# hmchuong/MaGGIe

Measured on AMD Instinct MI355X. Metric: instance-frames/sec (fwd+bwd+optimizer step, 512x512, bf16), higher is better.
Workload: dtype bf16

## Files before the change

### include/maggie_hip.h

```cpp
#ifndef MAGGIE_HIP_H
#define MAGGIE_HIP_H
#include <stdint.h>
#ifdef __cplusplus
extern "C" {
#endif

#define MG_F32 0
#define MG_BF16 1
#define MG_F16 3

#define MG_ACT_NONE 0
#define MG_ACT_RELU 1
#define MG_ACT_LRELU 2

#define MG_STAT_REPLICAS 32

#define MG_MODE_CONV 0
#define MG_MODE_TCONV 1
#define MG_MODE_GATHER 2

int mg_abi_version(void);
int mg_set_zeroed_range(void* base, long bytes);
int mg_zero_claim(void* p, long bytes);
int mg_zeroed_range_conflicts(void);
// ... 160 lines not shown
int mg_attn_tok_bwd(const float* p, const float* feat, const float* qk, const int32_t* ids, const float* dctx, const float* dp, int B, int T,
                    int L, int D, int NID, float scale, float* gbuf, float* rowdot, float* dqk, float* dbtab, float* dfeat, void* stream);
int mg_attn_feat_fwd(const float* feat, const float* kq, const float* b2, const float* vp, const float* obias, const uint8_t* pad_mask,
                     const int32_t* ids, int B, int T, int L, int D, int NID, float scale, float* out, float* p, void* stream);
int mg_attn_feat_bwd(const float* dout, const float* p, const float* feat, const float* kq, const float* vp, const int32_t* ids, int B, int T,
                     int L, int D, int NID, float scale, float* dfeat, float* dkq, float* dvp, float* db2, float* dobias, void* stream);
int mg_attn_feat_fwd_ex(const float* feat, const float* kq, const float* b2, const float* vp, const float* obias, const uint8_t* pad_mask,
                        const int32_t* ids, int B, int T, int L, int Dm, int NID, float scale, float* out, float* p, int b2_tn, void* stream);
int mg_attn_feat_bwd_ex(const float* dout, const float* p, const float* feat, const float* kq, const float* vp, const int32_t* ids, int B, int T,
                        int L, int Dm, int NID, float scale, float* dfeat, float* dkq, float* dvp, float* db2, float* dobias, int b2_tn, void* stream);

int mg_plane_flags(const float* w, int P, int HW, int32_t* flags, void* stream);
int mg_plane_flags_ex(const float* w, int P, int HW, void* flags, int as_float, void* stream);
int mg_os8_weight(const float* gt, const float* a8, int P, long HW, int reweight, int32_t* flags_scratch, float* out, void* stream);
int mg_os8_weight_ex(const float* gt, const float* a8, int P, long HW, int reweight, int32_t* flags_scratch, float* out, const int32_t* pvalid,
                     void* stream);
int mg_loss_finish(const float* sums, float* out3, void* stream);
int mg_loss_coef(const float* g3, const float* sums, float* coef5, void* stream);
int mg_loss_point_fwd(const float* p, const float* t, const float* w, const int32_t* flags, int P, int H, int W, float* d,
                      float* sums, const int32_t* pvalid, void* stream);
int mg_pyr_down(const float* x, const int32_t* flags, int P, int h, int w, float* out, void* stream);
int mg_pyr_lap_fwd(const float* x, const float* down, const float* w0, int lvl, int H0, int W0, const int32_t* flags, int P, int h,
                   int w, float* G, float* sums, void* stream);
int mg_pyr_upT(const float* q, const float* coef, const float* add, const int32_t* flags, int P, int h, int w, float* r, void* stream);
int mg_pyr_downT(const float* r, const float* q, const float* coef, const int32_t* flags, int P, int h, int w, float* dd, void* stream);
int mg_loss_point_bwd(const float* p, const float* t, const float* w, const int32_t* flags, int P, int H, int W, const float* coef_rec,
                      const float* coef_grad, const float* dd, float* A, float* B, float* dp, const int32_t* pvalid, void* stream);

int mg_matting_losses_fwd(const float* const* p, const float* t, const float* const* w, const int32_t* pvalid, int S, int P, int H, int W, int32_t* flags,
                          float* d, float* down0, float* down1, float* down2, float* G0, float* G1, float* G2, float* sums, float* out, void* stream);
int mg_matting_losses_bwd(const float* g, const float* sums, const float* const* p, const float* t, const float* const* w, const int32_t* pvalid,
                          const int32_t* flags, int S, int P, int H, int W, const float* G0, const float* G1, const float* G2, float* coef, float* r2,
                          float* dd2, float* r1, float* dd1, float* r0, float* dd0, float* A, float* B, float* dp, void* stream);

typedef struct mg_sn_desc {
    const float* W;
    float* u;
    float* v;
    int64_t out_off;
    int64_t work_off;
    int64_t dw_off;
    int32_t A, B, taps, transposed, pad_in;
    int32_t plain;
    int32_t k3_first, k3_count;
} mg_sn_desc;
int mg_spectral_norm_batched(const mg_sn_desc* descs, int n_conv, const int32_t* items_k1, int n1, const int32_t* items_k2, int n2,
                             const int32_t* items_k3, int n3, float* work_base, long work_floats, void* out_base, void* out_t_base,
                             int out_dtype, void* stream);
int mg_spectral_norm_batched_bwd(const mg_sn_desc* descs, int n_conv, const int32_t* items_k3, int n3, const void* const* Gptrs,
                                 int g_dtype, float* work_base, float* dW_base, float* dot_part, void* stream);
int mg_spectral_norm_batched_bwd_to(const mg_sn_desc* descs, int n_conv, const int32_t* items_k3, int n3, const void* const* Gptrs,
                                    int g_dtype, float* work_base, float* dW_base, float* const* dWptrs, float* dot_part, void* stream);

int mg_gru_gate_fwd(const void* rz, const void* x, const void* h, int dtype, int M, int C, void* xrh, void* stream);
int mg_gru_gate_bwd(const void* dxrh, const void* rz, const void* h, int dtype, int M, int C, void* dx, void* drz, void* dh_part, void* stream);
int mg_gru_out_fwd(const void* rz, const void* cpre, const void* h, int dtype, int M, int C, void* hn, void* stream);
int mg_gru_out_bwd(const void* dhn, const void* rz, const void* cpre, const void* h, int dtype, int M, int C, void* drz, void* dc_pre,
                   void* dh_part, void* stream);
int mg_temporal_fuse(float* alphas, const float* prev, const float* df, const float* db, long plane_elems, int n_frames, void* stream);

#define MG_WB_MAX_ENTRIES 64
typedef struct mg_wb_entry {
    const void* src;
    void* dst;
    void* dst_t;
    int32_t cout, taps, cin, cout_pad, cin_pad, flip_t, dtype, reserved;
// ... 399 lines not shown
```

### maggie_amd/csrc/loss_stencils.h

```cpp
#pragma once

MG_STENCIL_FN int st_refl(int k, int n) { return k < 0 ? -k : (k >= n ? 2 * (n - 1) - k : k); }
MG_STENCIL_FN int st_clampi(int k, int n) { return k < 0 ? 0 : (k >= n ? n - 1 : k); }

#define MG_G1 {1.f / 16.f, 4.f / 16.f, 6.f / 16.f, 4.f / 16.f, 1.f / 16.f}

MG_STENCIL_FN bool ring_map(int t, int nh, int nw, int T, int Bt, int Lw, int Rw, int& a, int& b) {
    const int hi = nh - T - Bt, wi = nw - Lw - Rw;
    if (hi <= 0 || wi <= 0) { a = t / nw; b = t - a * nw; return false; }
    const int n_int = hi * wi;
    if (t < n_int) { const int r = t / wi; a = T + r; b = Lw + (t - r * wi); return true; }
    int u = t - n_int;
    const int n_tb = (T + Bt) * nw;
    if (u < n_tb) { const int r = u / nw; a = r < T ? r : nh - Bt + (r - T); b = u - r * nw; return false; }
    u -= n_tb;
    const int side = Lw + Rw;
    const int r = u / side, k = u - r * side;
    a = T + r; b = k < Lw ? k : nw - Rw + (k - Lw);
    return false;
}

MG_STENCIL_FN float lap_up_general(const float* __restrict__ dp, int y, int xx, int h, int w, int wd) {
    const float g[5] = MG_G1;
    int yy[5], xs[5];
// ... 15 lines not shown
        }
        up += g[i] * r;
    }
    return up;
}
MG_STENCIL_FN void lap_up_inner(const float* __restrict__ dp, int a, int b, int wd, float* up) {
    const float* __restrict__ r0 = dp + (a - 1) * wd + (b - 1);
    float d[3][3];
#pragma unroll
    for (int r = 0; r < 3; ++r)
#pragma unroll
        for (int c = 0; c < 3; ++c) d[r][c] = r0[r * wd + c];
    const float g0 = 1.f / 16.f, g1 = 4.f / 16.f, g2 = 6.f / 16.f, g3 = 4.f / 16.f, g4 = 1.f / 16.f;
    float u = 0.f;
    u += g0 * (g0 * d[0][0] + g2 * d[0][1] + g4 * d[0][2]);
    u += g2 * (g0 * d[1][0] + g2 * d[1][1] + g4 * d[1][2]);
    u += g4 * (g0 * d[2][0] + g2 * d[2][1] + g4 * d[2][2]);
    up[0] = u;
    u = 0.f;
    u += g0 * (g1 * d[0][1] + g3 * d[0][2]);
    u += g2 * (g1 * d[1][1] + g3 * d[1][2]);
    u += g4 * (g1 * d[2][1] + g3 * d[2][2]);
    up[1] = u;
    u = 0.f;
    u += g1 * (g0 * d[1][0] + g2 * d[1][1] + g4 * d[1][2]);
    u += g3 * (g0 * d[2][0] + g2 * d[2][1] + g4 * d[2][2]);
    up[2] = u;
    u = 0.f;
    u += g1 * (g1 * d[1][1] + g3 * d[1][2]);
    u += g3 * (g1 * d[2][1] + g3 * d[2][2]);
    up[3] = u;
}

MG_STENCIL_FN float upT_general(const float* __restrict__ qp, int a, int b, int h, int w) {
    const float g[5] = MG_G1;
    float acc = 0.f;
#pragma unroll
    for (int sa = 0; sa < 3; ++sa) {
        int ma = sa == 0 ? 2 * a : (sa == 1 ? -2 * a : 2 * (h - 1) - 2 * a);
        if (sa == 1 && a != 1) continue;
        if (sa == 2 && ma != h) continue;
#pragma unroll
        for (int i = 0; i < 5; ++i) {
            int y = ma - i + 2;
            if (y < 0 || y >= h) continue;
            float v[3][5];
            bool ok[3][5];
#pragma unroll
            for (int sb = 0; sb < 3; ++sb) {
                const int mb = sb == 0 ? 2 * b : (sb == 1 ? -2 * b : 2 * (w - 1) - 2 * b);
                const bool on = !(sb == 1 && b != 1) && !(sb == 2 && mb != w);
#pragma unroll
                for (int j = 0; j < 5; ++j) {
                    const int xq = mb - j + 2;
                    ok[sb][j] = on && xq >= 0 && xq < w;
                    v[sb][j] = qp[y * w + (xq < 0 ? 0 : (xq >= w ? w - 1 : xq))];
                }
            }
            float rowacc = 0.f;
#pragma unroll
            for (int sb = 0; sb < 3; ++sb)
#pragma unroll
                for (int j = 0; j < 5; ++j) {
                    if (ok[sb][j]) rowacc += g[j] * v[sb][j];
                }
            acc += g[i] * rowacc;
// ... 94 lines not shown
            int x = X + dx;
            if (x < 0 || x >= W) continue;
            float av = Ap[y * W + x], bv = Bp[y * W + x];
#pragma unroll
            for (int i = 0; i < 3; ++i) {
                if (st_clampi(y + i - 1, H) != Y) continue;
#pragma unroll
                for (int j = 0; j < 3; ++j) {
                    if (st_clampi(x + j - 1, W) != X) continue;
                    acc += kx[i][j] * av + kx[j][i] * bv;
                }
            }
        }
    }
    return acc;
}
MG_STENCIL_FN float sobel_adj_inner(const float* __restrict__ Ap, const float* __restrict__ Bp, int Y, int X, int W) {
    const float kx[3][3] = {{-1.f, 0.f, 1.f}, {-2.f, 0.f, 2.f}, {-1.f, 0.f, 1.f}};
    float a[3][3], b[3][3];
#pragma unroll
    for (int dy = 0; dy < 3; ++dy)
#pragma unroll
        for (int dx = 0; dx < 3; ++dx) {
            a[dy][dx] = Ap[(Y + dy - 1) * W + (X + dx - 1)];
            b[dy][dx] = Bp[(Y + dy - 1) * W + (X + dx - 1)];
        }
    float acc = 0.f;
#pragma unroll
    for (int dy = 0; dy < 3; ++dy)
#pragma unroll
        for (int dx = 0; dx < 3; ++dx) acc += kx[2 - dy][2 - dx] * a[dy][dx] + kx[2 - dx][2 - dy] * b[dy][dx];
    return acc;
}
```

### maggie_amd/csrc/losses.hip

```cpp
#include "common.h"
#include "launch.h"
#include "../../include/maggie_hip.h"

namespace {

#define MG_STENCIL_FN __device__ __forceinline__
#include "loss_stencils.h"

constexpr int NT = 256;
__device__ __constant__ float c_g1[5] = {1.f / 16.f, 4.f / 16.f, 6.f / 16.f, 4.f / 16.f, 1.f / 16.f};

__device__ __forceinline__ int refl(int k, int n) { return k < 0 ? -k : (k >= n ? 2 * (n - 1) - k : k); }
__device__ __forceinline__ int clampi(int k, int n) { return k < 0 ? 0 : (k >= n ? n - 1 : k); }

constexpr int LOSS_REPLICAS = 32, LOSS_STRIDE = 16;
struct P3 { const float* a[3]; };
constexpr int LOSS_SUMS = LOSS_REPLICAS * LOSS_STRIDE;

__device__ __forceinline__ void block_add(float v, float* dst, float* sh, float* slot = nullptr) {
    v = wave_sum(v);
    const int lane = threadIdx.x & 63, wave = threadIdx.x >> 6;
    if (lane == 0) sh[wave] = v;
    __syncthreads();
    if (threadIdx.x == 0) {
// ... 34 lines not shown
    if (__syncthreads_or(any) && threadIdx.x == 0) flags[p] = 1;
}

__global__ __launch_bounds__(NT) void os8_weight_kernel(const float* __restrict__ gt, const float* __restrict__ a8, const int* __restrict__ flags,
                                                        long HW, int reweight, float* __restrict__ out, const int* __restrict__ pvalid) {
    const int p = blockIdx.y;
    const float valid = flags[p] ? 1.f : 0.f;
    const float pv = (pvalid && !pvalid[p]) ? 0.f : 1.f;
    const long base = (long)p * HW;
    const float lo = 1.0f / 255.0f, hi = 254.0f / 255.0f;
    for (long i = (long)blockIdx.x * NT + threadIdx.x; i < HW; i += (long)gridDim.x * NT) {
        float w = valid;
        if (reweight) {
            const float g = gt[base + i], a = a8[base + i] * pv;
            if ((g <= hi && g >= lo) || (a <= hi && a >= lo)) w += 1.f;
        }
        out[base + i] = w;
    }
}

__device__ __forceinline__ float sobel_mag(const float* __restrict__ a, const float* __restrict__ w, int y, int x, int H, int W, float& gx,
                                           float& gy, float as = 1.f) {
    float v[3][3];
#pragma unroll
    for (int i = 0; i < 3; ++i)
#pragma unroll
        for (int j = 0; j < 3; ++j) {
            int yy = clampi(y + i - 1, H), xx = clampi(x + j - 1, W);
            v[i][j] = a[yy * W + xx] * as * w[yy * W + xx];
        }
    gx = ((v[0][2] - v[0][0]) + 2.f * (v[1][2] - v[1][0]) + (v[2][2] - v[2][0])) * 0.125f;
    gy = ((v[2][0] - v[0][0]) + 2.f * (v[2][1] - v[0][1]) + (v[2][2] - v[0][2])) * 0.125f;
    return sqrtf(gx * gx + gy * gy + 1e-6f);
}

__global__ __launch_bounds__(NT) void point_fwd_kernel(const P3 p, const float* __restrict__ t, const P3 w,
                                                       const int* __restrict__ flags, int H, int W, float* __restrict__ d,
                                                       float* __restrict__ sums, const int* __restrict__ pvalid, int Pper, float* __restrict__ slots) {
    __shared__ float sh[NT / 64];
    const int pl = blockIdx.y;
    float* slot = slots ? slots + ((size_t)blockIdx.y * gridDim.x + blockIdx.x) * 3 : nullptr;
    if (!flags[pl]) { if (slot && threadIdx.x < 3) slot[threadIdx.x] = 0.f; return; }
    const int sc = pl / Pper, pq = pl - sc * Pper;
    const float pv = (pvalid && !pvalid[pq]) ? 0.f : 1.f;
    const long off = (long)pl * H * W, offq = (long)pq * H * W;
    const float *pp = p.a[sc] + offq, *tp = t + offq, *wp = w.a[sc] + offq;
    float s0 = 0.f, s1 = 0.f, s2 = 0.f;
    for (int i = blockIdx.x * NT + threadIdx.x; i < H * W; i += gridDim.x * NT) {
        int y = i / W, x = i - y * W;
        float dv = pp[i] * pv - tp[i], wv = wp[i];
        d[off + i] = dv;
        s0 += wv * fabsf(dv);
        s2 += wv;
        float gx, gy;
        float mp = sobel_mag(pp, wp, y, x, H, W, gx, gy, pv);
        float mt = sobel_mag(tp, wp, y, x, H, W, gx, gy);
        s1 += fabsf(mp - mt);
    }
    float* srep = sums + sc * LOSS_SUMS + ((blockIdx.y * gridDim.x + blockIdx.x) & (LOSS_REPLICAS - 1)) * LOSS_STRIDE;
    block_add(s0, &srep[0], sh, slot);
    block_add(s1, &srep[1], sh, slot ? slot + 1 : nullptr);
    block_add(s2, &srep[2], sh, slot ? slot + 2 : nullptr);
}

__global__ __launch_bounds__(NT) void pyr_down_kernel(const float* __restrict__ x, const int* __restrict__ flags, int h, int w,
                                                      float* __restrict__ out) {
// ... 41 lines not shown
            const float g1[5] = {1.f / 16.f, 4.f / 16.f, 6.f / 16.f, 4.f / 16.f, 1.f / 16.f};
            const int i0 = y & 1, j0 = xx & 1;
            const float* row = dp + ((y + i0 - 2) >> 1) * wd + ((xx + j0 - 2) >> 1);
            if (j0 == 0) {
                for (int i = i0; i < 5; i += 2, row += wd) up += g1[i] * (g1[0] * row[0] + g1[2] * row[1] + g1[4] * row[2]);
            } else {
                for (int i = i0; i < 5; i += 2, row += wd) up += g1[i] * (g1[1] * row[0] + g1[3] * row[1]);
            }
        } else {
#pragma unroll
            for (int i = 0; i < 5; ++i) {
                int yy = refl(y + i - 2, h);
                if (yy & 1) continue;
                float r = 0.f;
#pragma unroll
                for (int j = 0; j < 5; ++j) {
                    int xs = refl(xx + j - 2, w);
                    if (!(xs & 1)) r += c_g1[j] * dp[(yy >> 1) * wd + (xs >> 1)];
                }
                up += c_g1[i] * r;
            }
        }
        float L = xp[o] - 4.f * up;
        float wl = wp[(long)(y << lvl) * W0 + (xx << lvl)];
        s0 += fabsf(L) * wl;
        s1 += wl;
        G[(long)pl * h * w + o] = L > 0.f ? wl : (L < 0.f ? -wl : 0.f);
    }
    float* srep = sums + sc * LOSS_SUMS + ((blockIdx.y * gridDim.x + blockIdx.x) & (LOSS_REPLICAS - 1)) * LOSS_STRIDE;
    block_add(s0, &srep[0], sh, slot);
    block_add(s1, &srep[1], sh, slot ? slot + 1 : nullptr);
}

__global__ __launch_bounds__(NT) void pyr_upT_kernel(const float* __restrict__ q, const float* __restrict__ coef, const float* __restrict__ add,
                                                     const int* __restrict__ flags, int h, int w, float* __restrict__ r, int Pper) {
    const int pl = blockIdx.y;
    if (!flags[pl]) return;
    const int hd = h >> 1, wd = w >> 1;
    const float* qp = q + (long)pl * h * w;
    const float c = coef[(pl / Pper) * 5];
    for (int o = blockIdx.x * NT + threadIdx.x; o < hd * wd; o += gridDim.x * NT) {
        int a = o / wd, b = o - a * wd;
        float acc = 0.f;
#pragma unroll
        for (int sa = 0; sa < 3; ++sa) {
            int ma = sa == 0 ? 2 * a : (sa == 1 ? -2 * a : 2 * (h - 1) - 2 * a);
            if (sa == 1 && a != 1) continue;
            if (sa == 2 && ma != h) continue;
#pragma unroll
            for (int i = 0; i < 5; ++i) {
                int y = ma - i + 2;
                if (y < 0 || y >= h) continue;
                float rowacc = 0.f;
#pragma unroll
                for (int sb = 0; sb < 3; ++sb) {
                    int mb = sb == 0 ? 2 * b : (sb == 1 ? -2 * b : 2 * (w - 1) - 2 * b);
                    if (sb == 1 && b != 1) continue;
                    if (sb == 2 && mb != w) continue;
#pragma unroll
                    for (int j = 0; j < 5; ++j) {
                        int x = mb - j + 2;
                        if (x < 0 || x >= w) continue;
                        rowacc += c_g1[j] * qp[y * w + x];
                    }
                }
                acc += c_g1[i] * rowacc;
// ... 17 lines not shown
#pragma unroll
        for (int sa = 0; sa < 3; ++sa) {
            int my = sa == 0 ? Y : (sa == 1 ? -Y : 2 * (h - 1) - Y);
            if (sa == 1 && !(Y == 1 || Y == 2)) continue;
            if (sa == 2 && !(Y == h - 2 || Y == h - 3)) continue;
#pragma unroll
            for (int i = 0; i < 5; ++i) {
                int ty = my - i + 2;
                if (ty < 0 || (ty & 1)) continue;
                int y = ty >> 1;
                if (y >= hd) continue;
                float rowacc = 0.f;
#pragma unroll
                for (int sb = 0; sb < 3; ++sb) {
                    int mx = sb == 0 ? X : (sb == 1 ? -X : 2 * (w - 1) - X);
                    if (sb == 1 && !(X == 1 || X == 2)) continue;
                    if (sb == 2 && !(X == w - 2 || X == w - 3)) continue;
#pragma unroll
                    for (int j = 0; j < 5; ++j) {
                        int tx = mx - j + 2;
                        if (tx < 0 || (tx & 1)) continue;
                        int x = tx >> 1;
                        if (x >= wd) continue;
                        rowacc += c_g1[j] * rp[y * wd + x];
                    }
                }
                acc += c_g1[i] * rowacc;
            }
        }
        dd[(long)pl * h * w + o] = c * q[(long)pl * h * w + o] + acc;
    }
}

__global__ __launch_bounds__(NT) void pyr_lap_fwd_quad_kernel(const float* __restrict__ x, const float* __restrict__ down, const P3 w0,
                                                              int lvl, int H0, int W0, const int* __restrict__ flags, int h, int w,
                                                              float* __restrict__ G, float* __restrict__ sums, int Pper, float* __restrict__ slots) {
    __shared__ float sh[NT / 64];
    const int pl = blockIdx.y;
    float* slot = slots ? slots + ((size_t)blockIdx.y * gridDim.x + blockIdx.x) * 2 : nullptr;
    if (!flags[pl]) { if (slot && threadIdx.x < 2) slot[threadIdx.x] = 0.f; return; }
    const int sc = pl / Pper;
    const int hd = h >> 1, wd = w >> 1;
    const float* __restrict__ xp = x + (long)pl * h * w;
    const float* __restrict__ dp = down + (long)pl * hd * wd;
    const float* __restrict__ wp = w0.a[sc] + (long)(pl - sc * Pper) * H0 * W0;
    float* __restrict__ Gp = G + (long)pl * h * w;
    float s0 = 0.f, s1 = 0.f;
    const int hi = hd - 2, wi = wd - 2;
    const int n_int = (hi > 0 && wi > 0) ? hi * wi : 0;
    const int total = n_int + 4 * (hd * wd - n_int);
    for (int q = blockIdx.x * NT + threadIdx.x; q < total; q += gridDim.x * NT) {
        if (q >= n_int) {
            const int bt = q - n_int;
            int a, b;
            ring_map(n_int + (bt >> 2), hd, wd, 1, 1, 1, 1, a, b);
            const int y = 2 * a + ((bt >> 1) & 1), xx = 2 * b + (bt & 1);
            const float xv1 = xp[(long)y * w + xx];
            const float wl1 = wp[(long)(y << lvl) * W0 + (xx << lvl)];
            const float L = xv1 - 4.f * lap_up_general(dp, y, xx, h, w, wd);
            s0 += fabsf(L) * wl1;
            s1 += wl1;
            Gp[(long)y * w + xx] = L > 0.f ? wl1 : (L < 0.f ? -wl1 : 0.f);
            continue;
        }
        int a, b;
        ring_map(q, hd, wd, 1, 1, 1, 1, a, b);
        const int y0 = 2 * a, x0 = 2 * b;
        const float* __restrict__ xr0 = xp + (long)y0 * w + x0;
        const float xv[4] = {xr0[0], xr0[1], xr0[w], xr0[w + 1]};
        const long wr0 = (long)(y0 << lvl) * W0, wr1 = (long)((y0 + 1) << lvl) * W0;
        const int wc0 = x0 << lvl, wc1 = (x0 + 1) << lvl;
        const float wl[4] = {wp[wr0 + wc0], wp[wr0 + wc1], wp[wr1 + wc0], wp[wr1 + wc1]};
        float up[4];
        lap_up_inner(dp, a, b, wd, up);
        float gq[4];
#pragma unroll
        for (int u = 0; u < 4; ++u) {
            const float L = xv[u] - 4.f * up[u];
            s0 += fabsf(L) * wl[u];
            s1 += wl[u];
            gq[u] = L > 0.f ? wl[u] : (L < 0.f ? -wl[u] : 0.f);
        }
        float* __restrict__ gr0 = Gp + (long)y0 * w + x0;
        gr0[0] = gq[0]; gr0[1] = gq[1]; gr0[w] = gq[2]; gr0[w + 1] = gq[3];
    }
    float* srep = sums + sc * LOSS_SUMS + ((blockIdx.y * gridDim.x + blockIdx.x) & (LOSS_REPLICAS - 1)) * LOSS_STRIDE;
    block_add(s0, &srep[0], sh, slot);
    block_add(s1, &srep[1], sh, slot ? slot + 1 : nullptr);
}

__global__ __launch_bounds__(NT) void pyr_upT_batched_kernel(const float* __restrict__ q, const float* __restrict__ coef, const float* __restrict__ add,
                                                             const int* __restrict__ flags, int h, int w, float* __restrict__ r, int Pper) {
    const int pl = blockIdx.y;
    if (!flags[pl]) return;
    const int hd = h >> 1, wd = w >> 1;
    const float* __restrict__ qp = q + (long)pl * h * w;
    const float c = coef[(pl / Pper) * 5];
    for (int o = blockIdx.x * NT + threadIdx.x; o < hd * wd; o += gridDim.x * NT) {
        int a, b;
        const bool inner = ring_map(o, hd, wd, 2, 1, 2, 1, a, b);
        const long oo = (long)pl * hd * wd + a * wd + b;
        const float base = add ? add[oo] : 0.f;
        const float acc = inner ? upT_inner(qp, a, b, w) : upT_general(qp, a, b, h, w);
        r[oo] = base - 4.f * c * acc;
    }
}

__global__ __launch_bounds__(NT) void pyr_downT_quad_kernel(const float* __restrict__ r, const float* __restrict__ q, const float* __restrict__ coef,
                                                            const int* __restrict__ flags, int h, int w, float* __restrict__ dd, int Pper) {
    const int pl = blockIdx.y;
    if (!flags[pl]) return;
    const int hd = h >> 1, wd = w >> 1;
    const float* __restrict__ rp = r + (long)pl * hd * wd;
    const float* __restrict__ qp = q + (long)pl * h * w;
    float* __restrict__ op = dd + (long)pl * h * w;
    const float c = coef[(pl / Pper) * 5];
    const int hi = hd - 4, wi = wd - 4;
    const int n_int = (hi > 0 && wi > 0) ? hi * wi : 0;
    const int total = n_int + 4 * (hd * wd - n_int);
    for (int t = blockIdx.x * NT + threadIdx.x; t < total; t += gridDim.x * NT) {
        if (t >= n_int) {
            const int bt = t - n_int;
            int a, b;
            ring_map(n_int + (bt >> 2), hd, wd, 2, 2, 2, 2, a, b);
            const int Y = 2 * a + ((bt >> 1) & 1), X = 2 * b + (bt & 1);
            const float qv1 = qp[(long)Y * w + X];
            op[(long)Y * w + X] = c * qv1 + downT_general(rp, Y, X, h, w, hd, wd);
            continue;
        }
        int a, b;
        ring_map(t, hd, wd, 2, 2, 2, 2, a, b);
        const int y0 = 2 * a, x0 = 2 * b;
        const float* __restrict__ qr0 = qp + (long)y0 * w + x0;
        const float qv[4] = {qr0[0], qr0[1], qr0[w], qr0[w + 1]};
        float acc[4];
        downT_inner(rp, a, b, wd, acc);
        float* __restrict__ o0 = op + (long)y0 * w + x0;
        o0[0] = c * qv[0] + acc[0]; o0[1] = c * qv[1] + acc[1]; o0[w] = c * qv[2] + acc[2]; o0[w + 1] = c * qv[3] + acc[3];
    }
}

__global__ __launch_bounds__(NT) void sobel_bwd1_kernel(const P3 p, const float* __restrict__ t, const P3 w,
                                                        const int* __restrict__ flags, int H, int W, float* __restrict__ A, float* __restrict__ B,
                                                        const int* __restrict__ pvalid, int Pper) {
    const int pl = blockIdx.y;
    if (!flags[pl]) return;
    const int sc = pl / Pper, pq = pl - sc * Pper;
    if (pvalid && !pvalid[pq]) return;
    const long off = (long)pl * H * W, offq = (long)pq * H * W;
    const float *pp = p.a[sc] + offq, *tp = t + offq, *wp = w.a[sc] + offq;
    for (int i = blockIdx.x * NT + threadIdx.x; i < H * W; i += gridDim.x * NT) {
        int y = i / W, x = i - y * W;
        float gx, gy, tx, ty;
        float mp = sobel_mag(pp, wp, y, x, H, W, gx, gy);
        float mt = sobel_mag(tp, wp, y, x, H, W, tx, ty);
        float s = mp > mt ? 1.f : (mp < mt ? -1.f : 0.f);
        A[off + i] = s * gx / mp;
        B[off + i] = s * gy / mp;
    }
}

__global__ __launch_bounds__(NT) void point_bwd_kernel(const P3 p, const float* __restrict__ t, const P3 w,
                                                       const int* __restrict__ flags, int H, int W, const float* __restrict__ coef_rec,
                                                       const float* __restrict__ coef_grad, const float* __restrict__ dd,
                                                       const float* __restrict__ A, const float* __restrict__ B, float* __restrict__ dp,
                                                       const int* __restrict__ pvalid, int Pper) {
    const int pl = blockIdx.y;
    const int sc = pl / Pper, pq = pl - sc * Pper;
    const long off = (long)pl * H * W, offq = (long)pq * H * W;
    if (!flags[pl] || (pvalid && !pvalid[pq])) {
        for (int idx = blockIdx.x * NT + threadIdx.x; idx < H * W; idx += gridDim.x * NT) dp[off + idx] = 0.f;
        return;
    }
    const float cr = coef_rec[sc * 5], cg = coef_grad[sc * 5];
    const float* __restrict__ pp = p.a[sc] + offq;
    const float* __restrict__ tp = t + offq;
    const float* __restrict__ wp = w.a[sc] + offq;
    const float kx[3][3] = {{-1.f, 0.f, 1.f}, {-2.f, 0.f, 2.f}, {-1.f, 0.f, 1.f}};
    for (int idx = blockIdx.x * NT + threadIdx.x; idx < H * W; idx += gridDim.x * NT) {
        int Y = idx / W, X = idx - Y * W;
        float dv = pp[idx] - tp[idx];
        float wv = wp[idx];
        float g = cr * wv * (dv > 0.f ? 1.f : (dv < 0.f ? -1.f : 0.f));
        if (dd) g += dd[off + idx];
        float acc = 0.f;
#pragma unroll
        for (int dy = -1; dy <= 1; ++dy) {
            int y = Y + dy;
// ... 20 lines not shown

__global__ __launch_bounds__(NT) void point_bwd_batched_kernel(const P3 p, const float* __restrict__ t, const P3 w,
                                                               const int* __restrict__ flags, int H, int W, const float* __restrict__ coef_rec,
                                                               const float* __restrict__ coef_grad, const float* __restrict__ dd,
                                                               const float* __restrict__ A, const float* __restrict__ B, float* __restrict__ dp,
                                                               const int* __restrict__ pvalid, int Pper) {
    const int pl = blockIdx.y;
    const int sc = pl / Pper, pq = pl - sc * Pper;
    const long off = (long)pl * H * W, offq = (long)pq * H * W;
    if (!flags[pl] || (pvalid && !pvalid[pq])) {
        for (int idx = blockIdx.x * NT + threadIdx.x; idx < H * W; idx += gridDim.x * NT) dp[off + idx] = 0.f;
        return;
    }
    const float cr = coef_rec[sc * 5], cg = coef_grad[sc * 5];
    const float* __restrict__ pp = p.a[sc] + offq;
    const float* __restrict__ tp = t + offq;
    const float* __restrict__ wp = w.a[sc] + offq;
    const float* __restrict__ Ap = A + off;
    const float* __restrict__ Bp = B + off;
    for (int idx = blockIdx.x * NT + threadIdx.x; idx < H * W; idx += gridDim.x * NT) {
        int Y, X;
        const bool inner = ring_map(idx, H, W, 1, 1, 1, 1, Y, X);
        const int px = Y * W + X;
        const float dv = pp[px] - tp[px];
        const float wv = wp[px];
        const float ddv = dd ? dd[off + px] : 0.f;
        const float acc = inner ? sobel_adj_inner(Ap, Bp, Y, X, W) : sobel_adj_general(Ap, Bp, Y, X, H, W);
        float g = cr * wv * (dv > 0.f ? 1.f : (dv < 0.f ? -1.f : 0.f));
        if (dd) g += ddv;
        dp[off + px] = g + cg * wv * acc * 0.125f;
    }
}

inline dim3 grid2(long per_plane, int P, long max_blocks = 1024) {
    long b = (per_plane + NT - 1) / NT;
    if (b > max_blocks) b = max_blocks;
    if (b < 1) b = 1;
    return dim3((unsigned)b, (unsigned)P);
}
static const long REDUCING_BLOCKS_PER_PLANE = mg_env_long("MG_LOSS_BLOCKS", 256l);

static const int LOSS_BATCHED = (int)mg_env_long("MG_LOSS_BATCHED", 1);

static void launch_pyr_lap_fwd(dim3 g, hipStream_t st, const float* x, const float* down, P3 ww, int lvl, int H0, int W0, const int* flags, int h, int w,
                               float* G, float* sums, int Pper, float* slots) {
    if (LOSS_BATCHED && !(h & 1) && !(w & 1))
        hipLaunchKernelGGL(pyr_lap_fwd_quad_kernel, g, dim3(NT), 0, st, x, down, ww, lvl, H0, W0, flags, h, w, G, sums, Pper, slots);
    else
        hipLaunchKernelGGL(pyr_lap_fwd_kernel, g, dim3(NT), 0, st, x, down, ww, lvl, H0, W0, flags, h, w, G, sums, Pper, slots);
}
static void launch_pyr_upT(int SP, hipStream_t st, const float* q, const float* coef, const float* add, const int* flags, int h, int w, float* r, int Pper) {
    const dim3 g = grid2((long)(h / 2) * (w / 2), SP);
    if (LOSS_BATCHED && !(h & 1) && !(w & 1))
        hipLaunchKernelGGL(pyr_upT_batched_kernel, g, dim3(NT), 0, st, q, coef, add, flags, h, w, r, Pper);
    else
        hipLaunchKernelGGL(pyr_upT_kernel, g, dim3(NT), 0, st, q, coef, add, flags, h, w, r, Pper);
}
static void launch_pyr_downT(int SP, hipStream_t st, const float* r, const float* q, const float* coef, const int* flags, int h, int w, float* dd, int Pper) {
    if (LOSS_BATCHED && !(h & 1) && !(w & 1))
        hipLaunchKernelGGL(pyr_downT_quad_kernel, grid2((long)(h / 2) * (w / 2), SP), dim3(NT), 0, st, r, q, coef, flags, h, w, dd, Pper);
    else
        hipLaunchKernelGGL(pyr_downT_kernel, grid2((long)h * w, SP), dim3(NT), 0, st, r, q, coef, flags, h, w, dd, Pper);
}
static void launch_point_bwd(int SP, hipStream_t st, P3 pp, const float* t, P3 ww, const int* flags, int H, int W, const float* coef_rec,
                             const float* coef_grad, const float* dd, const float* A, const float* B, float* dp, const int* pvalid, int Pper) {
    if (LOSS_BATCHED)
        hipLaunchKernelGGL(point_bwd_batched_kernel, grid2((long)H * W, SP), dim3(NT), 0, st, pp, t, ww, flags, H, W, coef_rec, coef_grad, dd, A, B, dp, pvalid, Pper);
    else
        hipLaunchKernelGGL(point_bwd_kernel, grid2((long)H * W, SP), dim3(NT), 0, st, pp, t, ww, flags, H, W, coef_rec, coef_grad, dd, A, B, dp, pvalid, Pper);
}

__device__ __forceinline__ void loss_sum_replicas(const float* __restrict__ rep, float* s) {
    if (threadIdx.x < LOSS_STRIDE) {
        float a = 0.f;
        for (int r = 0; r < LOSS_REPLICAS; ++r) a += rep[r * LOSS_STRIDE + threadIdx.x];
// ... 135 lines not shown
extern "C" int mg_matting_losses_fwd(const float* const* p, const float* t, const float* const* w, const int32_t* pvalid, int S, int P, int H, int W,
                                     int32_t* flags, float* d, float* down0, float* down1, float* down2, float* G0, float* G1, float* G2, float* sums,
                                     float* out, void* stream) {
    if (S < 1 || S > 3 || P <= 0) return -2;
    if ((H & 7) || (W & 7) || H < 16 || W < 16) return -2;
    hipStream_t st = (hipStream_t)stream;
    P3 pp{{nullptr, nullptr, nullptr}}, ww{{nullptr, nullptr, nullptr}};
    for (int i = 0; i < S; ++i) { pp.a[i] = p[i]; ww.a[i] = w[i]; }
    const int SP = S * P;
    hipError_t e = mg_zero_words(flags, (long)SP, st); if (e != hipSuccess) return (int)e;
    e = mg_zero_words(sums, (long)S * LOSS_SUMS, st); if (e != hipSuccess) return (int)e;
    { dim3 g = grid2((long)H * W, SP); if (g.x > 64) g.x = 64; hipLaunchKernelGGL(plane_flags3_kernel, g, dim3(NT), 0, st, ww, P, H * W, flags); }
    {
        const dim3 g = grid2((long)H * W, SP, REDUCING_BLOCKS_PER_PLANE);
        float* slots; int rc = loss_slots(g, 3, &slots); if (rc) return rc;
        hipLaunchKernelGGL(point_fwd_kernel, g, dim3(NT), 0, st, pp, t, ww, flags, H, W, d, sums, pvalid, P, slots);
        rc = loss_slot_reduce(slots, g, S, 3, sums, 0, st); if (rc) return rc;
    }
    const float* x = d; float* downs[3] = {down0, down1, down2}; float* Gs[3] = {G0, G1, G2};
    int h = H, wd = W;
    for (int lvl = 0; lvl < 3; ++lvl) {
        hipLaunchKernelGGL(pyr_down_kernel, grid2((long)(h / 2) * (wd / 2), SP), dim3(NT), 0, st, x, flags, h, wd, downs[lvl]);
        const dim3 g = grid2((long)h * wd, SP, REDUCING_BLOCKS_PER_PLANE);
        float* slots; int rc = loss_slots(g, 2, &slots); if (rc) return rc;
        launch_pyr_lap_fwd(g, st, x, (const float*)downs[lvl], ww, lvl, H, W, flags, h, wd, Gs[lvl], sums + 3 + 2 * lvl, P, slots);
        rc = loss_slot_reduce(slots, g, S, 2, sums, 3 + 2 * lvl, st); if (rc) return rc;
        x = downs[lvl]; h >>= 1; wd >>= 1;
    }
    hipLaunchKernelGGL(loss_finish_kernel, dim3(S), dim3(64), 0, st, (const float*)sums, out);
    MG_CHECK_LAUNCH();
    return 0;
}

extern "C" int mg_matting_losses_bwd(const float* g, const float* sums, const float* const* p, const float* t, const float* const* w,
                                     const int32_t* pvalid, const int32_t* flags, int S, int P, int H, int W, const float* G0, const float* G1,
                                     const float* G2, float* coef, float* r2, float* dd2, float* r1, float* dd1, float* r0, float* dd0, float* A, float* B,
                                     float* dp, void* stream) {
    if (S < 1 || S > 3 || P <= 0) return -2;
    hipStream_t st = (hipStream_t)stream;
    P3 pp{{nullptr, nullptr, nullptr}}, ww{{nullptr, nullptr, nullptr}};
    for (int i = 0; i < S; ++i) { pp.a[i] = p[i]; ww.a[i] = w[i]; }
    const int SP = S * P;
    hipLaunchKernelGGL(loss_coef_kernel, dim3(S), dim3(64), 0, st, g, sums, coef);
    launch_pyr_upT(SP, st, G2, (const float*)(coef + 4), (const float*)nullptr, flags, H / 4, W / 4, r2, P);
    launch_pyr_downT(SP, st, (const float*)r2, G2, (const float*)(coef + 4), flags, H / 4, W / 4, dd2, P);
    launch_pyr_upT(SP, st, G1, (const float*)(coef + 3), (const float*)dd2, flags, H / 2, W / 2, r1, P);
    launch_pyr_downT(SP, st, (const float*)r1, G1, (const float*)(coef + 3), flags, H / 2, W / 2, dd1, P);
    launch_pyr_upT(SP, st, G0, (const float*)(coef + 2), (const float*)dd1, flags, H, W, r0, P);
    launch_pyr_downT(SP, st, (const float*)r0, G0, (const float*)(coef + 2), flags, H, W, dd0, P);
    hipLaunchKernelGGL(sobel_bwd1_kernel, grid2((long)H * W, SP), dim3(NT), 0, st, pp, t, ww, flags, H, W, A, B, pvalid, P);
    launch_point_bwd(SP, st, pp, t, ww, flags, H, W, (const float*)coef, (const float*)(coef + 1), (const float*)dd0, (const float*)A, (const float*)B, dp, pvalid, P);
    MG_CHECK_LAUNCH();
    return 0;
}

__global__ __launch_bounds__(NT) void atten_loss_rows_kernel(const float* __restrict__ gm, const float* __restrict__ att, long L, float* __restrict__ terms) {
    __shared__ float sh[2 * (NT / 64)];
    const long base = (long)blockIdx.x * L;
    float sv = 0.f, sg = 0.f;
    for (long i = threadIdx.x; i < L; i += NT) { const float g = gm[base + i]; sv += g * att[base + i]; sg += g; }
    sv = wave_sum(sv); sg = wave_sum(sg);
    const int lane = threadIdx.x & 63, wave = threadIdx.x >> 6;
    if (lane == 0) { sh[wave] = sv; sh[NT / 64 + wave] = sg; }
    __syncthreads();
    if (threadIdx.x == 0) {
        float a = 0.f, b = 0.f;
        for (int w = 0; w < NT / 64; ++w) { a += sh[w]; b += sh[NT / 64 + w]; }
        terms[blockIdx.x] = (b != 0.f ? 1.f : 0.f) - a;
    }
}
__global__ void atten_loss_sum_kernel(const float* __restrict__ terms, int rows, float scale, float* __restrict__ out) {
    float s = 0.f;
    for (int i = threadIdx.x; i < rows; i += 64) s += terms[i];
    s = wave_sum(s);
    if (threadIdx.x == 0) out[0] = s * scale;
}
// ... 45 lines not shown
```

### maggie_amd/functional.py

```python
import os

import torch
import torch.distributed as dist

from . import kernels as K
from .kernels import MODE_CONV, MODE_TCONV, MODE_GATHER, ACT_NONE, ACT_RELU, ACT_LRELU

LRELU_SLOPE = 0.2
import os as _os
UNFUSED_STATS_ROWS = int(_os.environ.get('MAGGIE_UNFUSED_STATS_ROWS', str(1 << 19)))
EXACT_STATS_ROWS = int(_os.environ.get('MAGGIE_EXACT_STATS_ROWS', '32768'))


class ZeroArena:

    def __init__(self):
        self.buf = None
        self.off = 0
        self.used = 0
        self.need = 1 << 20
        self.cap_buf = None
        self.cap_off = 0
        self.spills = 0
        self.tally = 0
# ... 1391 lines not shown
        t = target.detach().float().contiguous()
        P = ps[0].numel() // (H * W_)
        dev = t.device
        K.hip.need_cuda(t, *ps, *ws)
        if pvalid is not None:
            assert pvalid.dtype == torch.int32 and pvalid.numel() == P and pvalid.is_contiguous()
        SP = S * P
        new = lambda hh, ww: torch.empty((SP, hh, ww), dtype=torch.float32, device=dev)
        flags = ARENA.acc(SP, dev, torch.int32)
        sums = ARENA.acc(S * 512, dev)
        d, downs = new(H, W_), [new(H >> 1, W_ >> 1), new(H >> 2, W_ >> 2), new(H >> 3, W_ >> 3)]
        Gs = [new(H, W_), new(H >> 1, W_ >> 1), new(H >> 2, W_ >> 2)]
        out = torch.empty((S, 3), dtype=torch.float32, device=dev)
        parr = (K.ctypes.c_void_p * S)(*[x.data_ptr() for x in ps])
        warr = (K.ctypes.c_void_p * S)(*[x.data_ptr() for x in ws])
        ptr = K.hip.ptr
        K.hip.call('mg_matting_losses_fwd', parr, ptr(t), warr, ptr(pvalid), K.c_int(S), K.c_int(P), K.c_int(H), K.c_int(W_), ptr(flags), ptr(d),
                   ptr(downs[0]), ptr(downs[1]), ptr(downs[2]), ptr(Gs[0]), ptr(Gs[1]), ptr(Gs[2]), ptr(sums), ptr(out), K.hip.stream())
        ctx.save_for_backward(t, flags, sums, *Gs, *ps, *ws)
        ctx.pvalid, ctx.S, ctx.shape = pvalid, S, preds[0].shape
        return out

    @staticmethod
    def backward(ctx, g):
        S = ctx.S
        saved = ctx.saved_tensors
        t, flags, sums, G0, G1, G2 = saved[:6]
        ps, ws = saved[6:6 + S], saved[6 + S:6 + 2 * S]
        SP, H, W_ = G0.shape
        P = SP // S
        dev = t.device
        new = lambda hh, ww: torch.empty((SP, hh, ww), dtype=torch.float32, device=dev)
        coef = torch.empty((S, 5), dtype=torch.float32, device=dev)
        r2, dd2, r1, dd1 = new(H >> 3, W_ >> 3), new(H >> 2, W_ >> 2), new(H >> 2, W_ >> 2), new(H >> 1, W_ >> 1)
        r0, dd0, A, B, dp = new(H >> 1, W_ >> 1), new(H, W_), new(H, W_), new(H, W_), new(H, W_)
        parr = (K.ctypes.c_void_p * S)(*[x.data_ptr() for x in ps])
        warr = (K.ctypes.c_void_p * S)(*[x.data_ptr() for x in ws])
        ptr = K.hip.ptr
        K.hip.call('mg_matting_losses_bwd', ptr(g.float().contiguous()), ptr(sums), parr, ptr(t), warr, ptr(ctx.pvalid), ptr(flags), K.c_int(S), K.c_int(P),
                   K.c_int(H), K.c_int(W_), ptr(G0), ptr(G1), ptr(G2), ptr(coef), ptr(r2), ptr(dd2), ptr(r1), ptr(dd1), ptr(r0), ptr(dd0), ptr(A), ptr(B),
                   ptr(dp), K.hip.stream())
        dps = tuple(dp[i * P:(i + 1) * P].view(ctx.shape) for i in range(S))
        return (None, None) + dps + (None,) * S


def matting_losses_multi(preds, target, weights, pvalid=None):
    if not LOSS_MULTI or len(preds) == 1 or len(preds) > 3:
        return [matting_losses(p_, target, w_, pvalid) for p_, w_ in zip(preds, weights)]
    out = MattingLossesMulti.apply(target, pvalid, *preds, *weights)
    cells = SplitGrid.apply(out)
    n = out.shape[1]
    return [cells[i * n:(i + 1) * n] for i in range(out.shape[0])]


class SplitGrid(torch.autograd.Function):

    @staticmethod
    def forward(ctx, t):
        ctx.set_materialize_grads(False)
        ctx.shape = t.shape
        return tuple(t[i, j] for i in range(t.shape[0]) for j in range(t.shape[1]))

    @staticmethod
    def backward(ctx, *gs):
        R, C = ctx.shape
        g0 = gs[0]
        if g0 is not None and all(g is not None and g.dtype == torch.float32 and g.numel() == 1 and g.is_cuda and
                                  g.untyped_storage().data_ptr() == g0.untyped_storage().data_ptr() and g.data_ptr() == g0.data_ptr() + 4 * i
# ... 698 lines not shown
```

Measured before the change: 773.6.

## Fuse matting-loss backward pyramid transposes and Sobel/point gradient into tiled kernels

Replaces the separate upT/downT launches of the Laplacian-pyramid backward with a combined updownT kernel per level. It also fuses the Sobel adjoint (A/B maps) and point-loss backward into one shared-memory tiled kernel that stages pred, target and weight tiles with halos. This removes intermediate dd and A/B buffers along with several kernel launches and full-resolution memory round trips. The cost is more complex tiled code with halo recomputation, plus FP-contraction pragmas intended to keep rounding consistent with the unfused path.

Result: no change. 767.2 (-0.8%).

```diff
diff --git a/include/maggie_hip.h b/include/maggie_hip.h
--- a/include/maggie_hip.h
+++ b/include/maggie_hip.h
@@ -216,6 +216,8 @@
 int mg_matting_losses_bwd(const float* g, const float* sums, const float* const* p, const float* t, const float* const* w, const int32_t* pvalid,
                           const int32_t* flags, int S, int P, int H, int W, const float* G0, const float* G1, const float* G2, float* coef, float* r2,
                           float* dd2, float* r1, float* dd1, float* r0, float* dd0, float* A, float* B, float* dp, void* stream);
+int mg_set_loss_fused(int on);
+int mg_matting_losses_bwd_fused(int H, int W);
 
 typedef struct mg_sn_desc {
     const float* W;
diff --git a/maggie_amd/csrc/loss_stencils.h b/maggie_amd/csrc/loss_stencils.h
--- a/maggie_amd/csrc/loss_stencils.h
+++ b/maggie_amd/csrc/loss_stencils.h
@@ -71,6 +71,10 @@
     up[3] = u;
 }
 
+#if defined(__clang__)
+#pragma clang fp contract(on)
+#endif
+
 MG_STENCIL_FN float upT_general(const float* __restrict__ qp, int a, int b, int h, int w) {
     const float g[5] = MG_G1;
     float acc = 0.f;
@@ -231,3 +235,148 @@
         for (int dx = 0; dx < 3; ++dx) acc += kx[2 - dy][2 - dx] * a[dy][dx] + kx[2 - dx][2 - dy] * b[dy][dx];
     return acc;
 }
+MG_STENCIL_FN float sobel_adj_general_at(const float* __restrict__ Ap, const float* __restrict__ Bp, int Y, int X, int H, int W, int oy, int ox,
+                                         int stride) {
+    const float kx[3][3] = {{-1.f, 0.f, 1.f}, {-2.f, 0.f, 2.f}, {-1.f, 0.f, 1.f}};
+    float acc = 0.f;
+#pragma unroll
+    for (int dy = -1; dy <= 1; ++dy) {
+        int y = Y + dy;
+        if (y < 0 || y >= H) continue;
+#pragma unroll
+        for (int dx = -1; dx <= 1; ++dx) {
+            int x = X + dx;
+            if (x < 0 || x >= W) continue;
+            float av = Ap[(y - oy) * stride + (x - ox)], bv = Bp[(y - oy) * stride + (x - ox)];
+#pragma unroll
+            for (int i = 0; i < 3; ++i) {
+                if (st_clampi(y + i - 1, H) != Y) continue;
+#pragma unroll
+                for (int j = 0; j < 3; ++j) {
+                    if (st_clampi(x + j - 1, W) != X) continue;
+                    acc += kx[i][j] * av + kx[j][i] * bv;
+                }
+            }
+        }
+    }
+    return acc;
+}
+
+MG_STENCIL_FN float sobel_mag9(const float (&a)[3][3], const float (&w)[3][3], float as, float& gx, float& gy) {
+#if defined(__clang__)
+#pragma clang fp contract(off)
+#endif
+#define MG_SOBEL_D(i1, j1, i0, j0) fmaf(a[i1][j1] * as, w[i1][j1], -((a[i0][j0] * as) * w[i0][j0]))
+    gx = ((MG_SOBEL_D(0, 2, 0, 0) + 2.f * MG_SOBEL_D(1, 2, 1, 0)) + MG_SOBEL_D(2, 2, 2, 0)) * 0.125f;
+    gy = ((MG_SOBEL_D(2, 0, 0, 0) + 2.f * MG_SOBEL_D(2, 1, 0, 1)) + MG_SOBEL_D(2, 2, 0, 2)) * 0.125f;
+#undef MG_SOBEL_D
+    const float g2 = gx * gx, h2 = gy * gy;
+    return sqrtf((g2 + h2) + 1e-6f);
+}
+
+constexpr int LF_T = 32, LF_NT = 256;
+constexpr int LF_SS = LF_T + 4;
+constexpr int LF_RS = LF_T + 2;
+MG_STENCIL_FN int lf_tiles(int n) { return (n + LF_T - 1) / LF_T; }
+MG_STENCIL_FN int lf_extent(int o0, int n) { return n - o0 < LF_T ? n - o0 : LF_T; }
+
+MG_STENCIL_FN void lf_stage(int tid, const float* __restrict__ pp, const float* __restrict__ tp, const float* __restrict__ wp, int Y0, int X0, int H,
+                            int W, float* __restrict__ s_p, float* __restrict__ s_t, float* __restrict__ s_w) {
+    const int sh = lf_extent(Y0, H) + 4, sw = lf_extent(X0, W) + 4;
+    for (int l = tid; l < sh * sw; l += LF_NT) {
+        const int ly = l / sw, lx = l - ly * sw;
+        const int g = st_clampi(Y0 - 2 + ly, H) * W + st_clampi(X0 - 2 + lx, W);
+        s_p[ly * LF_SS + lx] = pp[g];
+        s_t[ly * LF_SS + lx] = tp[g];
+        s_w[ly * LF_SS + lx] = wp[g];
+    }
+}
+
+MG_STENCIL_FN float sobel_mag_window(const float* __restrict__ a, const float* __restrict__ w, int o, int stride, float& gx, float& gy, float as = 1.f) {
+    float va[3][3], vw[3][3];
+#pragma unroll
+    for (int i = 0; i < 3; ++i)
+#pragma unroll
+        for (int j = 0; j < 3; ++j) { va[i][j] = a[o + i * stride + j]; vw[i][j] = w[o + i * stride + j]; }
+    return sobel_mag9(va, vw, as, gx, gy);
+}
+
+MG_STENCIL_FN void lf_ring(int tid, const float* __restrict__ s_p, const float* __restrict__ s_t, const float* __restrict__ s_w, int Y0, int X0, int H,
+                           int W, float* __restrict__ s_A, float* __restrict__ s_B) {
+    const int rh = lf_extent(Y0, H) + 2, rw = lf_extent(X0, W) + 2;
+    for (int l = tid; l < rh * rw; l += LF_NT) {
+        const int ry = l / rw, rx = l - ry * rw;
+        const int y = Y0 - 1 + ry, x = X0 - 1 + rx;
+        float a = 0.f, b = 0.f;
+        if (y >= 0 && y < H && x >= 0 && x < W) {
+            float gx, gy, tx, ty;
+            const float mp = sobel_mag_window(s_p, s_w, ry * LF_SS + rx, LF_SS, gx, gy);
+            const float mt = sobel_mag_window(s_t, s_w, ry * LF_SS + rx, LF_SS, tx, ty);
+            const float s = mp > mt ? 1.f : (mp < mt ? -1.f : 0.f);
+            a = s * gx / mp;
+            b = s * gy / mp;
+        }
+        s_A[ry * LF_RS + rx] = a;
+        s_B[ry * LF_RS + rx] = b;
+    }
+}
+
+MG_STENCIL_FN float lf_dpred(float pv, float tv, float wv, float cr, float cg, float ddv, float adj) {
+    const float dv = pv - tv;
+    float g = cr * wv * (dv > 0.f ? 1.f : (dv < 0.f ? -1.f : 0.f));
+    g += ddv;
+    return g + cg * wv * adj * 0.125f;
+}
+
+MG_STENCIL_FN void lf_apply(int tid, const float* __restrict__ pp, const float* __restrict__ tp, const float* __restrict__ wp,
+                            const float* __restrict__ qp, const float* __restrict__ rp, const float* __restrict__ s_A,
+                            const float* __restrict__ s_B, int Y0, int X0, int H, int W, float cr, float cg, float c, float* __restrict__ op) {
+    const int qy = tid / (LF_T / 2), qx = tid - qy * (LF_T / 2);
+    const int y0 = Y0 + 2 * qy, x0 = X0 + 2 * qx;
+    if (y0 >= H || x0 >= W) return;
+    const int hd = H >> 1, wd = W >> 1, a = y0 >> 1, b = x0 >> 1;
+    const long o00 = (long)y0 * W + x0;
+    const long o[4] = {o00, o00 + 1, o00 + W, o00 + W + 1};
+    float pv[4], tv[4], wv[4], qv[4], acc[4], adj[4];
+#pragma unroll
+    for (int u = 0; u < 4; ++u) { pv[u] = pp[o[u]]; tv[u] = tp[o[u]]; wv[u] = wp[o[u]]; qv[u] = qp[o[u]]; }
+    if (hd - 4 > 0 && wd - 4 > 0 && a >= 2 && a < hd - 2 && b >= 2 && b < wd - 2) {
+        downT_inner(rp, a, b, wd, acc);
+    } else {
+#pragma unroll
+        for (int u = 0; u < 4; ++u) acc[u] = downT_general(rp, y0 + (u >> 1), x0 + (u & 1), H, W, hd, wd);
+    }
+#pragma unroll
+    for (int u = 0; u < 4; ++u) {
+        const int y = y0 + (u >> 1), x = x0 + (u & 1);
+        const int ry = y - (Y0 - 1), rx = x - (X0 - 1);
+        adj[u] = (y >= 1 && y < H - 1 && x >= 1 && x < W - 1) ? sobel_adj_inner(s_A, s_B, ry, rx, LF_RS)
+                                                              : sobel_adj_general_at(s_A, s_B, y, x, H, W, Y0 - 1, X0 - 1, LF_RS);
+    }
+#pragma unroll
+    for (int u = 0; u < 4; ++u) op[o[u]] = lf_dpred(pv[u], tv[u], wv[u], cr, cg, c * qv[u] + acc[u], adj[u]);
+}
+
+MG_STENCIL_FN int lf_ud_total(int hd, int wd) {
+    const int hi = hd - 4, wi = wd - 4;
+    const int n_int = (hi > 0 && wi > 0) ? hi * wi : 0;
+    return n_int + 4 * (hd * wd - n_int);
+}
+MG_STENCIL_FN bool lf_ud_map(int t, int hd, int wd, int& Y, int& X) {
+    const int hi = hd - 4, wi = wd - 4;
+    const int n_int = (hi > 0 && wi > 0) ? hi * wi : 0;
+    int a, b;
+    if (t < n_int) { ring_map(t, hd, wd, 2, 2, 2, 2, a, b); Y = 2 * a; X = 2 * b; return true; }
+    const int bt = t - n_int;
+    ring_map(n_int + (bt >> 2), hd, wd, 2, 2, 2, 2, a, b);
+    Y = 2 * a + ((bt >> 1) & 1); X = 2 * b + (bt & 1);
+    return false;
+}
+MG_STENCIL_FN float lf_upT_cell(const float* __restrict__ up, int a, int b, int h, int w) {
+    const bool inner = h - 3 > 0 && w - 3 > 0 && a >= 2 && a < h - 1 && b >= 2 && b < w - 1;
+    return inner ? upT_inner(up, a, b, 2 * w) : upT_general(up, a, b, 2 * h, 2 * w);
+}
+
+#if defined(__clang__)
+#pragma clang fp contract(fast)
+#endif
diff --git a/maggie_amd/csrc/losses.hip b/maggie_amd/csrc/losses.hip
--- a/maggie_amd/csrc/losses.hip
+++ b/maggie_amd/csrc/losses.hip
@@ -90,6 +90,19 @@
     gx = ((v[0][2] - v[0][0]) + 2.f * (v[1][2] - v[1][0]) + (v[2][2] - v[2][0])) * 0.125f;
     gy = ((v[2][0] - v[0][0]) + 2.f * (v[2][1] - v[0][1]) + (v[2][2] - v[0][2])) * 0.125f;
     return sqrtf(gx * gx + gy * gy + 1e-6f);
+}
+__device__ __forceinline__ float sobel_mag_bwd(const float* __restrict__ a, const float* __restrict__ w, int y, int x, int H, int W, float& gx,
+                                               float& gy) {
+    float va[3][3], vw[3][3];
+#pragma unroll
+    for (int i = 0; i < 3; ++i)
+#pragma unroll
+        for (int j = 0; j < 3; ++j) {
+            int yy = clampi(y + i - 1, H), xx = clampi(x + j - 1, W);
+            va[i][j] = a[yy * W + xx];
+            vw[i][j] = w[yy * W + xx];
+        }
+    return sobel_mag9(va, vw, 1.f, gx, gy);
 }
 
 __global__ __launch_bounds__(NT) void point_fwd_kernel(const P3 p, const float* __restrict__ t, const P3 w,
@@ -197,6 +210,7 @@
     block_add(s1, &srep[1], sh, slot ? slot + 1 : nullptr);
 }
 
+#pragma clang fp contract(on)
 __global__ __launch_bounds__(NT) void pyr_upT_kernel(const float* __restrict__ q, const float* __restrict__ coef, const float* __restrict__ add,
                                                      const int* __restrict__ flags, int h, int w, float* __restrict__ r, int Pper) {
     const int pl = blockIdx.y;
@@ -280,6 +294,7 @@
     }
 }
 
+#pragma clang fp contract(fast)
 __global__ __launch_bounds__(NT) void pyr_lap_fwd_quad_kernel(const float* __restrict__ x, const float* __restrict__ down, const P3 w0,
                                                               int lvl, int H0, int W0, const int* __restrict__ flags, int h, int w,
                                                               float* __restrict__ G, float* __restrict__ sums, int Pper, float* __restrict__ slots) {
@@ -337,6 +352,7 @@
     block_add(s1, &srep[1], sh, slot ? slot + 1 : nullptr);
 }
 
+#pragma clang fp contract(on)
 __global__ __launch_bounds__(NT) void pyr_upT_batched_kernel(const float* __restrict__ q, const float* __restrict__ coef, const float* __restrict__ add,
                                                              const int* __restrict__ flags, int h, int w, float* __restrict__ r, int Pper) {
     const int pl = blockIdx.y;
@@ -400,8 +416,8 @@
     for (int i = blockIdx.x * NT + threadIdx.x; i < H * W; i += gridDim.x * NT) {
         int y = i / W, x = i - y * W;
         float gx, gy, tx, ty;
-        float mp = sobel_mag(pp, wp, y, x, H, W, gx, gy);
-        float mt = sobel_mag(tp, wp, y, x, H, W, tx, ty);
+        float mp = sobel_mag_bwd(pp, wp, y, x, H, W, gx, gy);
+        float mt = sobel_mag_bwd(tp, wp, y, x, H, W, tx, ty);
         float s = mp > mt ? 1.f : (mp < mt ? -1.f : 0.f);
         A[off + i] = s * gx / mp;
         B[off + i] = s * gy / mp;
@@ -488,6 +504,78 @@
     }
 }
 
+__global__ __launch_bounds__(NT) void pyr_updownT_kernel(const float* __restrict__ r, const float* __restrict__ q, const float* __restrict__ coef,
+                                                         const float* __restrict__ qup, const float* __restrict__ coef_up,
+                                                         const int* __restrict__ flags, int h, int w, float* __restrict__ rout, int Pper) {
+    const int pl = blockIdx.y;
+    if (!flags[pl]) return;
+    const int hd = h >> 1, wd = w >> 1;
+    const float* __restrict__ rp = r + (long)pl * hd * wd;
+    const float* __restrict__ qp = q + (long)pl * h * w;
+    const float* __restrict__ up = qup + (long)pl * h * w * 4;
+    float* __restrict__ op = rout + (long)pl * h * w;
+    const float c = coef[(pl / Pper) * 5], cu = coef_up[(pl / Pper) * 5];
+    const int total = lf_ud_total(hd, wd);
+    for (int t = blockIdx.x * NT + threadIdx.x; t < total; t += gridDim.x * NT) {
+        int Y, X;
+        if (!lf_ud_map(t, hd, wd, Y, X)) {
+            const float base = c * qp[(long)Y * w + X] + downT_general(rp, Y, X, h, w, hd, wd);
+            op[(long)Y * w + X] = base - 4.f * cu * lf_upT_cell(up, Y, X, h, w);
+            continue;
+        }
+        const float* __restrict__ qr0 = qp + (long)Y * w + X;
+        const float qv[4] = {qr0[0], qr0[1], qr0[w], qr0[w + 1]};
+        float acc[4], ut[4];
+        downT_inner(rp, Y >> 1, X >> 1, wd, acc);
+#pragma unroll
+        for (int u = 0; u < 4; ++u) ut[u] = lf_upT_cell(up, Y + (u >> 1), X + (u & 1), h, w);
+        float* __restrict__ o0 = op + (long)Y * w + X;
+        float base[4];
+#pragma unroll
+        for (int u = 0; u < 4; ++u) base[u] = c * qv[u] + acc[u];
+        o0[0] = base[0] - 4.f * cu * ut[0]; o0[1] = base[1] - 4.f * cu * ut[1];
+        o0[w] = base[2] - 4.f * cu * ut[2]; o0[w + 1] = base[3] - 4.f * cu * ut[3];
+    }
+}
+
+__global__ __launch_bounds__(LF_NT) void point_bwd_fused_kernel(const P3 p, const float* __restrict__ t, const P3 w, const int* __restrict__ flags,
+                                                                int H, int W, const float* __restrict__ coef, const float* __restrict__ G0,
+                                                                const float* __restrict__ r0, float* __restrict__ dp,
+                                                                const int* __restrict__ pvalid, int Pper) {
+    __shared__ float s_p[LF_SS * LF_SS], s_t[LF_SS * LF_SS], s_w[LF_SS * LF_SS], s_A[LF_RS * LF_RS], s_B[LF_RS * LF_RS];
+    const int pl = blockIdx.y;
+    const int sc = pl / Pper, pq = pl - sc * Pper;
+    const int tx = lf_tiles(W);
+    const int Y0 = (blockIdx.x / tx) * LF_T, X0 = (blockIdx.x % tx) * LF_T;
+    const long off = (long)pl * H * W, offq = (long)pq * H * W;
+    if (!flags[pl] || (pvalid && !pvalid[pq])) {
+        const int th = lf_extent(Y0, H), tw = lf_extent(X0, W);
+        if (!((uintptr_t)dp & 15)) {
+            const int tw4 = tw >> 2;
+            for (int l = threadIdx.x; l < th * tw4; l += LF_NT) {
+                const int ly = l / tw4, lx = l - ly * tw4;
+                *reinterpret_cast<float4*>(dp + off + (long)(Y0 + ly) * W + X0 + 4 * lx) = make_float4(0.f, 0.f, 0.f, 0.f);
+            }
+        } else {
+            for (int l = threadIdx.x; l < th * tw; l += LF_NT) {
+                const int ly = l / tw, lx = l - ly * tw;
+                dp[off + (long)(Y0 + ly) * W + X0 + lx] = 0.f;
+            }
+        }
+        return;
+    }
+    const float* __restrict__ pp = p.a[sc] + offq;
+    const float* __restrict__ tp = t + offq;
+    const float* __restrict__ wp = w.a[sc] + offq;
+    lf_stage(threadIdx.x, pp, tp, wp, Y0, X0, H, W, s_p, s_t, s_w);
+    __syncthreads();
+    lf_ring(threadIdx.x, s_p, s_t, s_w, Y0, X0, H, W, s_A, s_B);
+    __syncthreads();
+    lf_apply(threadIdx.x, pp, tp, wp, G0 + off, r0 + (long)pl * (H >> 1) * (W >> 1), s_A, s_B, Y0, X0, H, W, coef[sc * 5], coef[sc * 5 + 1],
+             coef[sc * 5 + 2], dp + off);
+}
+
+#pragma clang fp contract(fast)
 inline dim3 grid2(long per_plane, int P, long max_blocks = 1024) {
     long b = (per_plane + NT - 1) / NT;
     if (b > max_blocks) b = max_blocks;
@@ -497,6 +585,7 @@
 static const long REDUCING_BLOCKS_PER_PLANE = mg_env_long("MG_LOSS_BLOCKS", 256l);
 
 static const int LOSS_BATCHED = (int)mg_env_long("MG_LOSS_BATCHED", 1);
+static int g_loss_fused = (int)mg_env_long("MG_LOSS_FUSED", 1) ? 1 : 0;
 
 static void launch_pyr_lap_fwd(dim3 g, hipStream_t st, const float* x, const float* down, P3 ww, int lvl, int H0, int W0, const int* flags, int h, int w,
                                float* G, float* sums, int Pper, float* slots) {
@@ -698,6 +787,11 @@
     return 0;
 }
 
+extern "C" int mg_matting_losses_bwd_fused(int H, int W) {
+    return g_loss_fused && LOSS_BATCHED && !(H & 7) && !(W & 7) && H >= 16 && W >= 16;
+}
+extern "C" int mg_set_loss_fused(int on) { const int was = g_loss_fused; g_loss_fused = on ? 1 : 0; return was; }
+
 extern "C" int mg_matting_losses_bwd(const float* g, const float* sums, const float* const* p, const float* t, const float* const* w,
                                      const int32_t* pvalid, const int32_t* flags, int S, int P, int H, int W, const float* G0, const float* G1,
                                      const float* G2, float* coef, float* r2, float* dd2, float* r1, float* dd1, float* r0, float* dd0, float* A, float* B,
@@ -707,7 +801,20 @@
     P3 pp{{nullptr, nullptr, nullptr}}, ww{{nullptr, nullptr, nullptr}};
     for (int i = 0; i < S; ++i) { pp.a[i] = p[i]; ww.a[i] = w[i]; }
     const int SP = S * P;
+    const int fused = mg_matting_losses_bwd_fused(H, W);
+    if (!fused && (!dd2 || !dd1 || !dd0 || !A || !B)) return -2;
     hipLaunchKernelGGL(loss_coef_kernel, dim3(S), dim3(64), 0, st, g, sums, coef);
+    if (fused) {
+        launch_pyr_upT(SP, st, G2, (const float*)(coef + 4), (const float*)nullptr, flags, H / 4, W / 4, r2, P);
+        hipLaunchKernelGGL(pyr_updownT_kernel, grid2((long)(H / 8) * (W / 8), SP), dim3(NT), 0, st, (const float*)r2, G2, (const float*)(coef + 4), G1,
+                           (const float*)(coef + 3), flags, H / 4, W / 4, r1, P);
+        hipLaunchKernelGGL(pyr_updownT_kernel, grid2((long)(H / 4) * (W / 4), SP), dim3(NT), 0, st, (const float*)r1, G1, (const float*)(coef + 3), G0,
+                           (const float*)(coef + 2), flags, H / 2, W / 2, r0, P);
+        hipLaunchKernelGGL(point_bwd_fused_kernel, dim3((unsigned)(((H + LF_T - 1) / LF_T) * ((W + LF_T - 1) / LF_T)), (unsigned)SP), dim3(LF_NT), 0, st, pp, t, ww, flags, H, W,
+                           (const float*)coef, G0, (const float*)r0, dp, pvalid, P);
+        MG_CHECK_LAUNCH();
+        return 0;
+    }
     launch_pyr_upT(SP, st, G2, (const float*)(coef + 4), (const float*)nullptr, flags, H / 4, W / 4, r2, P);
     launch_pyr_downT(SP, st, (const float*)r2, G2, (const float*)(coef + 4), flags, H / 4, W / 4, dd2, P);
     launch_pyr_upT(SP, st, G1, (const float*)(coef + 3), (const float*)dd2, flags, H / 2, W / 2, r1, P);
diff --git a/maggie_amd/functional.py b/maggie_amd/functional.py
--- a/maggie_amd/functional.py
+++ b/maggie_amd/functional.py
@@ -1447,8 +1447,11 @@
         dev = t.device
         new = lambda hh, ww: torch.empty((SP, hh, ww), dtype=torch.float32, device=dev)
         coef = torch.empty((S, 5), dtype=torch.float32, device=dev)
-        r2, dd2, r1, dd1 = new(H >> 3, W_ >> 3), new(H >> 2, W_ >> 2), new(H >> 2, W_ >> 2), new(H >> 1, W_ >> 1)
-        r0, dd0, A, B, dp = new(H >> 1, W_ >> 1), new(H, W_), new(H, W_), new(H, W_), new(H, W_)
+        r2, r1, r0, dp = new(H >> 3, W_ >> 3), new(H >> 2, W_ >> 2), new(H >> 1, W_ >> 1), new(H, W_)
+        if K.hip.lib().mg_matting_losses_bwd_fused(K.c_int(H), K.c_int(W_)):
+            dd2 = dd1 = dd0 = A = B = None
+        else:
+            dd2, dd1, dd0, A, B = new(H >> 2, W_ >> 2), new(H >> 1, W_ >> 1), new(H, W_), new(H, W_), new(H, W_)
         parr = (K.ctypes.c_void_p * S)(*[x.data_ptr() for x in ps])
         warr = (K.ctypes.c_void_p * S)(*[x.data_ptr() for x in ws])
         ptr = K.hip.ptr
```
